# zilliztech/knowhere

Hardware: NVIDIA H100
Metric: queries/sec at recall@10>=0.95, 10Mx128 f32 IVF_PQ (higher is better)
Workload: dtype f32

## Files before the change

### knowhere_b200/csrc/kb2_ivfpq_tc.cuh

```cuda
#pragma once
#include <cuda_bf16.h>

#include <type_traits>
#include <utility>

#include "kb2_gemm_tc.cuh"
#include "kb2_ivf.cuh"
#include "kb2_listmajor.cuh"

namespace kb2 {
namespace pqtc {

using lm::TM;
constexpr int NQT = 256;
constexpr int THREADS = 512;
constexpr int GROUP_THREADS = 128;
constexpr int MAXW = 80;
constexpr int META_BYTES = 3 * NQT * 4;
template <int G, int DSUB>
struct TcCfg {
    static constexpr int M = 16 * G;
    static constexpr int KD = M * DSUB;
    static_assert(KD % 16 == 0 && (DSUB == 2 || DSUB == 4 || DSUB == 8), "unsupported PQ geometry");
    static constexpr int XCHUNK = KD / 8;
    static constexpr int KSTEPS = KD / 16 + 1;
    static constexpr int CHUNKS = 2 * KSTEPS;
    static constexpr int GRP_BYTES = CHUNKS * 128;
    static constexpr int TAB_BYTES = M * 256 * DSUB * 2;
    static constexpr int A_BYTES = (TM / 8) * GRP_BYTES, B_BYTES = (NQT / 8) * GRP_BYTES;
    static constexpr int OFF_TAB = 0;
    static constexpr int OFF_A = TAB_BYTES;
    static constexpr int OFF_B = OFF_A + 2 * A_BYTES;
    static constexpr int OFF_META = OFF_B + B_BYTES;
    static constexpr int OFF_BAR = OFF_META + 2 * META_BYTES;
    static constexpr size_t SMEM_BYTES = OFF_BAR + 256 + 128 ;
    static_assert(SMEM_BYTES <= 227 * 1024, "filter kernel shared memory");
};
constexpr int KD = 128;
constexpr float kErrCoef = 0.0085f;
constexpr float kAccCoef = 4e-5f;

struct Params {
    int metric;
    int nq, nprobe;
    const float* queries;
    const __nv_bfloat16* qb16;
    const float* qnorm;
    const int32_t* n_items;
    int32_t* ticket;
    const int32_t* item_list;
    const int32_t* item_q0;
    const int32_t* item_nq;
    const int32_t* pair_q;
    const float* pair_base;
    const float* bound;
    int k_need;
    float margin_coef;
    float rmax;
    const int64_t* list_off;
    const int32_t* list_len;
    const uint4* codes;
    const uint4* codes_plain;
    int64_t npad;
    const float* t1;
    const float* pqc;
    const uint4* pqc16;
    const uint8_t* bitset;
    const int32_t* rows;
    uint4* log;
    uint32_t* log_cnt;
    uint32_t log_cap;
    uint32_t* qflag;
    unsigned long long* counters;
};

template <typename F, int... I>
__device__ __forceinline__ void
static_for_impl(F&& f, std::integer_sequence<int, I...>) {
    (f(std::integral_constant<int, I>{}), ...);
}
template <int N, typename F>
__device__ __forceinline__ void
static_for(F&& f) {
    static_for_impl(f, std::make_integer_sequence<int, N>{});
}
template <int C0_, int W_>
struct BlockCols {
    static constexpr int C0 = C0_, W = W_;
};
template <int LO, int HI, typename F>
__device__ __forceinline__ void
dispatch_range(int n, F&& f) {
    if constexpr (LO == HI) {
        f(std::integral_constant<int, LO>{});
    } else {
        constexpr int MID = (LO + HI) / 2;
        if (n <= MID) dispatch_range<LO, MID>(n, f);
        else dispatch_range<MID + 1, HI>(n, f);
    }
}

__device__ __forceinline__ void
bar_sync_epi() {
    asm volatile("bar.sync 1, 256;" ::: "memory");
}
__device__ __forceinline__ uint64_t
make_desc_ns(uint32_t smem_addr, uint32_t grp_bytes) {
    uint64_t d = 0;
    d |= (uint64_t)((smem_addr & 0x3FFFFu) >> 4);
    d |= (uint64_t)(128 >> 4) << 16;
    d |= (uint64_t)(grp_bytes >> 4) << 32;
    return d;
}

#ifdef KB2_FILTER_STALLS
#define KB2_STALL_BEGIN(v) const long long v = clock64()
#define KB2_STALL_END(slot, v) stall[slot] += clock64() - (v)
constexpr int kStallMaxCtas = 1024, kStallSlots = 8;
__device__ unsigned long long g_filter_stalls[kStallMaxCtas][2][2][kStallSlots];
__global__ void
filter_stalls_print_kernel(int ctas) {
    for (int b = 0; b < min(ctas, kStallMaxCtas); b++) {
        printf("KB2STALL cta=%d", b);
        for (int r = 0; r < 2; r++) {
            printf(r == 0 ? " dec=" : " cons=");
            for (int i = 0; i < kStallSlots; i++)
                printf(i ? ",%llu" : "%llu", g_filter_stalls[b][r][0][i] + g_filter_stalls[b][r][1][i]);
        }
        printf("\n");
    }
}
#else
#define KB2_STALL_BEGIN(v)
#define KB2_STALL_END(slot, v)
#endif

__device__ __forceinline__ void
split3_bf16(float x, uint32_t& hi, uint32_t& mid, uint32_t& lo) {
    const __nv_bfloat16 h = __float2bfloat16_rn(x);
    hi = (uint32_t)__bfloat16_as_ushort(h);
    if (!(fabsf(x) < INFINITY)) { mid = 0u; lo = 0u; return; }
    const float r1 = x - __bfloat162float(h);
    const __nv_bfloat16 m = __float2bfloat16_rn(r1);
    const float r2 = r1 - __bfloat162float(m);
    mid = (uint32_t)__bfloat16_as_ushort(m);
    lo = (uint32_t)__bfloat16_as_ushort(__float2bfloat16_rn(r2));
}

template <int METRIC, int G, int DSUB>
__global__ void __launch_bounds__(THREADS, 1)
ivfpq_tc_filter_kernel(Params p) {
    using C = TcCfg<G, DSUB>;
    constexpr int KD = C::KD, XCHUNK = C::XCHUNK, KSTEPS = C::KSTEPS, GRP_BYTES = C::GRP_BYTES, TAB_BYTES = C::TAB_BYTES;
    constexpr int A_BYTES = C::A_BYTES, OFF_TAB = C::OFF_TAB, OFF_A = C::OFF_A, OFF_B = C::OFF_B, OFF_META = C::OFF_META,
                  OFF_BAR = C::OFF_BAR;
    extern __shared__ unsigned char smem_dyn[];
    const uint32_t raw = tc::smem_u32(smem_dyn);
    const uint32_t base = (raw + 127u) & ~127u;
    unsigned char* sm = smem_dyn + (base - raw);
    const uint32_t bars = base + OFF_BAR;
    auto bar_a_full = [&](int i) { return bars + 8u * i; };
    auto bar_a_empty = [&](int i) { return bars + 8u * (2 + i); };
    const uint32_t bar_b_full = bars + 8u * 8, bar_b_free = bars + 8u * 9;
    auto bar_meta_full = [&](int i) { return bars + 8u * (10 + i); };
    auto bar_meta_free = [&](int i) { return bars + 8u * (12 + i); };
    uint32_t* qcnt = (uint32_t*)(sm + OFF_BAR + 8 * 15);

    const int warp = __shfl_sync(0xffffffffu, (int)threadIdx.x >> 5, 0), lane = threadIdx.x & 31;
    const int n_items = *p.n_items;

    const lm::ItemRing<8> ring(sm + OFF_BAR + 144, p.ticket);
    ring.init();

    if (threadIdx.x == 0) {
        for (int i = 0; i < 2; i++) {
            tc::mbar_init(bar_a_full(i), GROUP_THREADS);
            tc::mbar_init(bar_a_empty(i), GROUP_THREADS);
            tc::mbar_init(bar_meta_full(i), 2 * GROUP_THREADS);
            tc::mbar_init(bar_meta_free(i), 2 * GROUP_THREADS);
        }
        tc::mbar_init(bar_b_full, 2 * GROUP_THREADS);
        tc::mbar_init(bar_b_free, 2 * GROUP_THREADS);
        qcnt[0] = qcnt[1] = qcnt[2] = qcnt[3] = 0;
        asm volatile("fence.mbarrier_init.release.cluster;" ::: "memory");
    }
#ifdef KB2_FILTER_STALLS
    long long stall[kStallSlots] = {0, 0, 0, 0, 0, 0, 0, 0};
    KB2_STALL_BEGIN(t_role);
#endif
    {
        uint4* tab = (uint4*)(sm + OFF_TAB);
        for (int i = threadIdx.x; i < TAB_BYTES / 16; i += THREADS) tab[i] = __ldg(p.pqc16 + i);
    }
    __syncthreads();
    const float inv_alpha = (METRIC == KB2_METRIC_L2) ? 0.5f : 1.f;

    if (warp < 8) {
        const int dt = threadIdx.x;
        const int dg = dt >> 7;
        const int tid = dt & 127;
        const uint4* tab = (const uint4*)(sm + OFF_TAB);
        auto write_meta = [&](int item, int it) {
            KB2_STALL_BEGIN(t_meta);
            const int par = it & 1;
            tc::mbar_wait(bar_meta_free(par), (((uint32_t)it >> 1) & 1u) ^ 1u);
            const int q0 = p.item_q0[item];
            const int nqi = p.item_nq[item];
            float* m_h = (float*)(sm + OFF_META + par * META_BYTES);
            float* m_base = m_h + NQT;
            int* m_q = (int*)(m_base + NQT);
            const int j = dt;
            float h = -INFINITY, bs = 0.f;
            int q = -1;
            if (j < nqi) {
                q = p.pair_q[q0 + j];
                bs = p.pair_base[q0 + j];
                const float bnd = p.bound[q];
                if (!(bnd < INFINITY)) {
                    p.qflag[q] = 1u;
                    if (p.counters) atomicAdd(p.counters + 6, 1ull << 32);
                } else {
                    const float margin = p.margin_coef * p.qnorm[q] * 1.01f + 1e-30f;
                    const float h0 = (bnd + margin - bs) * inv_alpha;
                    h = h0 + kAccCoef * (fabsf(h0) + p.rmax) + 1e-30f;
                }
            }
            m_h[j] = h;
            m_base[j] = bs;
            m_q[j] = q;
            tc::mbar_arrive(bar_meta_full(par));
            KB2_STALL_END(5, t_meta);
        };
        uint32_t g0 = 0;
        int it = 0;
        int item = ring.at_warp(0);
        if (item < n_items) write_meta(item, 0);
        for (; item < n_items; it++) {
            const int item_next = ring.at_warp(it + 1);
            const int l = p.item_list[item];
            const int nqi = p.item_nq[item];
            const int nmma = (nqi + 15) & ~15;
            const int len = p.list_len[l];
            const int64_t off = p.list_off[l];
            const int ntiles = (len + TM - 1) / TM;
            const int par = it & 1;
            const int t_first = (int)((dg - (int)(g0 & 1u)) & 1);
            uint4 w_next[G];
#pragma unroll
            for (int g = 0; g < G; g++) w_next[g] = make_uint4(0, 0, 0, 0);
            float t_next = 0.f;
            const uint4* code_src = (DSUB == 8) ? p.codes : p.codes_plain;
            if (t_first < ntiles && off + (int64_t)t_first * TM + tid < p.npad) {
#pragma unroll
                for (int g = 0; g < G; g++) w_next[g] = ldg_stream_u4(code_src + (int64_t)g * p.npad + off + (int64_t)t_first * TM + tid);
                if (METRIC == KB2_METRIC_L2) t_next = __ldg(p.t1 + off + (int64_t)t_first * TM + tid);
            }
            auto decode_tile = [&](int t) {
                KB2_STALL_BEGIN(t_dec);
                const uint32_t g = g0 + (uint32_t)t;
                uint4 w[G];
#pragma unroll
                for (int gg = 0; gg < G; gg++) w[gg] = w_next[gg];
                const float tv = t_next;
                {
                    const int64_t pn = off + (int64_t)(t + 2) * TM + tid;
                    if (t + 2 < ntiles && pn < p.npad) {
#pragma unroll
                        for (int gg = 0; gg < G; gg++) w_next[gg] = ldg_stream_u4(code_src + (int64_t)gg * p.npad + pn);
                        if (METRIC == KB2_METRIC_L2) t_next = __ldg(p.t1 + pn);
                    }
                }
                float r = INFINITY;
                if (t * TM + tid < len) r = (METRIC == KB2_METRIC_L2) ? 0.5f * tv : 0.f;
                uint32_t rh, rm, rl;
                split3_bf16(-r, rh, rm, rl);
                uint4 v[XCHUNK];
                if constexpr (DSUB == 8) {
#pragma unroll
                    for (int gg = 0; gg < G; gg++) {
                        const uint32_t ww[4] = {w[gg].x, w[gg].y, w[gg].z, w[gg].w};
#pragma unroll
                        for (int s = 0; s < 16; s++) {
                            const uint32_t byte = (ww[s >> 2] >> (8 * (s & 3))) & 255u;
                            v[gg * 16 + s] = tab[byte * (16 * G) + gg * 16 + ((s + tid) & 15)];
                        }
                    }
                } else {
                    constexpr int SPC = 8 / DSUB;
                    constexpr int WPS = DSUB / 2;
                    const uint32_t* tab32 = reinterpret_cast<const uint32_t*>(tab);
#pragma unroll
                    for (int c = 0; c < XCHUNK; c++) {
                        uint32_t u[4];
#pragma unroll
                        for (int j = 0; j < SPC; j++) {
                            const int m = c * SPC + j;
                            const uint4 wg = w[m >> 4];
                            const int b = m & 15;
                            const uint32_t word = (b < 4) ? wg.x : (b < 8) ? wg.y : (b < 12) ? wg.z : wg.w;
                            const uint32_t byte = (word >> (8 * (b & 3))) & 255u;
#pragma unroll
                            for (int x = 0; x < WPS; x++) u[j * WPS + x] = tab32[(m * 256 + byte) * WPS + x];
                        }
                        v[c] = make_uint4(u[0], u[1], u[2], u[3]);
                    }
                }
                KB2_STALL_BEGIN(t_ae);
                tc::mbar_wait(bar_a_empty(dg), ((g >> 1) & 1u) ^ 1u);
                KB2_STALL_END(1, t_ae);
                unsigned char* A = sm + OFF_A + dg * A_BYTES + (tid >> 3) * GRP_BYTES + (tid & 7) * 16;
#pragma unroll
                for (int c = 0; c < XCHUNK; c++) {
                    const int chunk = (DSUB == 8) ? (c & ~15) + ((c + tid) & 15) : c;
                    *reinterpret_cast<uint4*>(A + chunk * 128) = v[c];
                }
                *reinterpret_cast<uint4*>(A + XCHUNK * 128) = make_uint4(rh | (rm << 16), rl | (0x3F80u << 16), 0x3F803F80u, 0u);
                *reinterpret_cast<uint4*>(A + (XCHUNK + 1) * 128) = make_uint4(0u, 0u, 0u, 0u);
                tc::fence_proxy_async();
                tc::mbar_arrive(bar_a_full(dg));
                KB2_STALL_END(3, t_dec);
            };
            if (t_first < ntiles) decode_tile(t_first);
            KB2_STALL_BEGIN(t_b);
            asm volatile("bar.sync 2, 256;" ::: "memory");
            KB2_STALL_BEGIN(t_bf);
            tc::mbar_wait(bar_b_free, ((uint32_t)it & 1u) ^ 1u);
            KB2_STALL_END(2, t_bf);
            {
                const float* m_h = (const float*)(sm + OFF_META + par * META_BYTES);
                const int* m_q = (const int*)(m_h + 2 * NQT);
                const uint32_t Bs = base + OFF_B;
                unsigned char* B = sm + OFF_B;
                const int kc = tid >> 3;
                const int rsub = tid & 7;
                for (int blk = dg; blk < nmma / 8 && kc < XCHUNK; blk += 2) {
                    const int row = blk * 8 + rsub;
                    const int q = m_q[row];
                    const uint32_t dst = (uint32_t)(blk * GRP_BYTES + kc * 128 + rsub * 16);
                    if (q >= 0) {
                        const void* src = reinterpret_cast<const uint4*>(p.qb16 + (int64_t)q * KD) + kc;
                        asm volatile("cp.async.cg.shared.global [%0], [%1], 16;" ::"r"(Bs + dst), "l"(src) : "memory");
                    } else {
                        *reinterpret_cast<uint4*>(B + dst) = make_uint4(0, 0, 0, 0);
                    }
                }
                if (dt < nmma) {
                    uint32_t hh, hm, hl;
                    split3_bf16(m_h[dt], hh, hm, hl);
                    unsigned char* Bc = B + (dt >> 3) * GRP_BYTES + (dt & 7) * 16;
                    *reinterpret_cast<uint4*>(Bc + XCHUNK * 128) = make_uint4(0x3F803F80u, 0x3F80u | (hh << 16), hm | (hl << 16), 0u);
                    *reinterpret_cast<uint4*>(Bc + (XCHUNK + 1) * 128) = make_uint4(0u, 0u, 0u, 0u);
                }
                asm volatile("cp.async.wait_all;" ::: "memory");
            }
            tc::fence_proxy_async();
            tc::mbar_arrive(bar_b_full);
            KB2_STALL_END(4, t_b);
            if (item_next < n_items) write_meta(item_next, it + 1);
            for (int t = t_first + 2; t < ntiles; t += 2) decode_tile(t);
            g0 += (uint32_t)ntiles;
            item = item_next;
        }
    } else {
        const int et = threadIdx.x - 256;
        const int eg = et >> 7;
        const int e = et & 127;
        const int we = warp & 3;
        const uint32_t n_logs = 2u * gridDim.x;
        uint4* my_log = p.log + (size_t)(2 * blockIdx.x + eg) * p.log_cap;
        uint32_t* my_cursor = qcnt + eg;
        bool log_over = false;
        unsigned long long n_codes = 0;
        uint32_t g0 = 0;
        int it = 0;
        for (int item = ring.at_warp(0); item < n_items; item = ring.at_warp(++it)) {
            const int l = p.item_list[item];
            const int nqi = p.item_nq[item];
            const int ncls = __shfl_sync(0xffffffffu, (nqi + 15) >> 4, 0);
            const int len = p.list_len[l];
            const int64_t off = p.list_off[l];
            const int ntiles = (len + TM - 1) / TM;
            const int par = it & 1;
            KB2_STALL_BEGIN(t_mf);
            tc::mbar_wait(bar_meta_full(par), ((uint32_t)it >> 1) & 1u);
            KB2_STALL_END(1, t_mf);
            const float* m_base = (const float*)(sm + OFF_META + par * META_BYTES) + NQT;
            const int* m_q = (const int*)(m_base + NQT);
            if (et == 0) n_codes += (unsigned long long)len * (unsigned long long)nqi;
            const int t_first = (int)((eg - (int)(g0 & 1u)) & 1);
            KB2_STALL_BEGIN(t_bfull);
            tc::mbar_wait(bar_b_full, (uint32_t)it & 1u);
            KB2_STALL_END(2, t_bfull);
            const uint32_t a0 = base + OFF_A + eg * A_BYTES;
            const uint32_t b0 = base + OFF_B;
            const uint32_t la0 = (uint32_t)make_desc_ns(a0, GRP_BYTES), lb0 = (uint32_t)make_desc_ns(b0, GRP_BYTES);
            constexpr uint64_t desc_hi = (uint64_t)(GRP_BYTES >> 4) << 32;
            for (int t = t_first; t < ntiles; t += 2) {
                const uint32_t g = g0 + (uint32_t)t;
                KB2_STALL_BEGIN(t_af);
                tc::mbar_wait(bar_a_full(eg), (g >> 1) & 1u);
                KB2_STALL_END(3, t_af);
                auto issue = [&](auto& acc, int h, auto blk) {
                    using B = decltype(blk);
                    KB2_STALL_BEGIN(t_is);
                    uint32_t la = la0 + (uint32_t)(h * 8 * GRP_BYTES / 16), lb = lb0 + (uint32_t)(B::C0 / 8 * GRP_BYTES / 16);
                    if constexpr (G == 1) asm volatile("" : "+r"(la), "+r"(lb));
                    tc::fence_operand(acc);
                    tc::wgmma_fence();
#pragma unroll
                    for (int ks = 0; ks < KSTEPS; ks++)
                        tc::wgmma_bf16<B::W>(acc, desc_hi | (la + ks * 16u), desc_hi | (lb + ks * 16u), ks > 0 ? 1u : 0u);
                    tc::wgmma_commit();
                    tc::fence_operand(acc);
                    KB2_STALL_END(6, t_is);
                };
                uint64_t mh[2][2] = {{0ull, 0ull}, {0ull, 0ull}};
                auto test = [&](const auto& v, int h, auto blk) {
                    using B = decltype(blk);
                    constexpr int NBIT = B::W / 4, HALF = NBIT / 2;
                    KB2_STALL_BEGIN(t_te);
                    uint32_t n0l = 0u, n0h = 0u, n1l = 0u, n1h = 0u;
#pragma unroll
                    for (int i = HALF - 1; i >= 0; i--) {
                        const int x = 4 * (i >> 1) + (i & 1);
                        const int xh = 4 * ((i + HALF) >> 1) + ((i + HALF) & 1);
                        n0l = __funnelshift_l(__float_as_uint(v[x]), n0l, 1);
                        n0h = __funnelshift_l(__float_as_uint(v[xh]), n0h, 1);
                        n1l = __funnelshift_l(__float_as_uint(v[x + 2]), n1l, 1);
                        n1h = __funnelshift_l(__float_as_uint(v[xh + 2]), n1h, 1);
                    }
                    constexpr uint32_t mask = (1u << NBIT) - 1u;
                    const uint32_t m0 = ~((n0h << HALF) | n0l) & mask, m1 = ~((n1h << HALF) | n1l) & mask;
                    mh[h][0] |= (uint64_t)m0 << (B::C0 / 4);
                    mh[h][1] |= (uint64_t)m1 << (B::C0 / 4);
                    KB2_STALL_END(7, t_te);
                };
                auto flush = [&]() {
                    const uint32_t total =
                        (uint32_t)(__popcll(mh[0][0]) + __popcll(mh[0][1]) + __popcll(mh[1][0]) + __popcll(mh[1][1]));
                    if (total != 0u) {
                        uint32_t slot = atomicAdd(my_cursor, total);
#pragma unroll
                        for (int h = 0; h < 2; h++) {
#pragma unroll
                            for (int i = 0; i < 2; i++) {
                                const int rel = t * TM + h * 64 + we * 16 + (lane >> 2) + 8 * i;
                                uint64_t m = mh[h][i];
                                while (m) {
                                    const int bit = __ffsll((long long)m) - 1;
                                    m &= m - 1;
                                    const int col = 8 * (bit >> 1) + 2 * (lane & 3) + (bit & 1);
                                    if (slot < p.log_cap) {
                                        uint4 o;
                                        o.x = (uint32_t)m_q[col];
                                        o.y = (uint32_t)(off + rel);
                                        o.z = __float_as_uint(m_base[col]);
                                        o.w = 0u;
                                        my_log[slot] = o;
                                    } else {
                                        log_over = true;
                                    }
                                    slot++;
                                }
                            }
                        }
                    }
                };
                dispatch_range<1, NQT / 16>(ncls, [&](auto nc) {
                    constexpr int NC = decltype(nc)::value, NB = (16 * NC + MAXW - 1) / MAXW, NBT = 2 * NB;
                    constexpr int U = NC / NB, X = NC % NB;
                    auto blk = [](auto cc) {
                        constexpr int c = decltype(cc)::value;
                        return BlockCols<16 * (c * U + (c < X ? c : X)), 16 * (U + (c < X ? 1 : 0))>{};
                    };
                    float va[8 * (U + (X > 0 ? 1 : 0))], vb[8 * (U + (X > 0 ? 1 : 0))];
                    issue(va, 0, blk(std::integral_constant<int, 0>{}));
                    static_for<NBT>([&](auto bc) {
                        constexpr int b = decltype(bc)::value;
                        if constexpr (b + 1 < NBT) {
                            constexpr auto bn = blk(std::integral_constant<int, (b + 1) % NB>{});
                            if constexpr ((b + 1) & 1) issue(vb, (b + 1) / NB, bn);
                            else issue(va, (b + 1) / NB, bn);
                            KB2_STALL_BEGIN(t_w);
                            tc::wgmma_wait<1>();
                            KB2_STALL_END(4, t_w);
                        } else {
                            KB2_STALL_BEGIN(t_w);
                            tc::wgmma_wait<0>();
                            KB2_STALL_END(4, t_w);
                        }
                        constexpr auto bb = blk(std::integral_constant<int, b % NB>{});
                        if constexpr (b & 1) {
                            tc::fence_operand(vb);
                            test(vb, b / NB, bb);
                        } else {
                            tc::fence_operand(va);
                            test(va, b / NB, bb);
                        }
                    });
                });
                tc::mbar_arrive(bar_a_empty(eg));
                KB2_STALL_BEGIN(t_fl);
                flush();
                KB2_STALL_END(5, t_fl);
            }
            tc::mbar_arrive(bar_b_free);
            tc::mbar_arrive(bar_meta_free(par));
            g0 += (uint32_t)ntiles;
        }
        if (log_over) p.log_cnt[n_logs] = 1u;
        if (eg == 0) asm volatile("bar.sync 3, 128;" ::: "memory"); else asm volatile("bar.sync 4, 128;" ::: "memory");
        if (e == 0) {
            const uint32_t n = min(*my_cursor, p.log_cap);
            p.log_cnt[2 * blockIdx.x + eg] = n;
            if (p.counters) atomicAdd(p.counters + 2, (unsigned long long)n);
        }
        if (et == 0 && p.counters) atomicAdd(p.counters, n_codes);
    }
#ifdef KB2_FILTER_STALLS
    KB2_STALL_END(0, t_role);
    if ((threadIdx.x & 127) == 0 && blockIdx.x < kStallMaxCtas) {
        for (int i = 0; i < kStallSlots; i++)
            g_filter_stalls[blockIdx.x][warp >= 8][(threadIdx.x >> 7) & 1][i] = (unsigned long long)stall[i];
    }
#endif
}

__global__ void
prepare_queries_kernel(const float* __restrict__ q, int64_t nq, int d, __nv_bfloat16* __restrict__ qb16, float* __restrict__ qnorm) {
    const int64_t w = ((int64_t)blockIdx.x * blockDim.x + threadIdx.x) >> 5;
    const int lane = threadIdx.x & 31;
    if (w >= nq) return;
    float s = 0.f;
    for (int j = lane * 4; j < d; j += 128) {
        const float4 v = __ldg(reinterpret_cast<const float4*>(q + w * d + j));
        __nv_bfloat162 lo = __floats2bfloat162_rn(v.x, v.y), hi = __floats2bfloat162_rn(v.z, v.w);
        uint2 o;
        o.x = *reinterpret_cast<uint32_t*>(&lo);
        o.y = *reinterpret_cast<uint32_t*>(&hi);
        *reinterpret_cast<uint2*>(qb16 + w * d + j) = o;
        s += v.x * v.x + v.y * v.y + v.z * v.z + v.w * v.w;
    }
    s = warp_sum(s);
    if (lane == 0) qnorm[w] = sqrtf(s) * 1.0001f;
}

__global__ void __launch_bounds__(256)
prepare_tables_kernel(const float* __restrict__ pqc, int dsub, __nv_bfloat16* __restrict__ pqc16, float* __restrict__ maxn2) {
    const int m = blockIdx.x, j = threadIdx.x;
    const int M = gridDim.x;
    const float* c = pqc + ((size_t)m * 256 + j) * dsub;
    float n2 = 0.f;
    __nv_bfloat16* o = pqc16 + (dsub == 8 ? ((size_t)j * M + m) : ((size_t)m * 256 + j)) * dsub;
    for (int t = 0; t < dsub; t++) {
        n2 = fmaf(c[t], c[t], n2);
        o[t] = __float2bfloat16_rn(c[t]);
    }
    __shared__ float red[256];
    red[j] = n2;
    __syncthreads();
    for (int s = 128; s > 0; s >>= 1) {
        if (j < s) red[j] = fmaxf(red[j], red[j + s]);
        __syncthreads();
    }
    if (j == 0) maxn2[m] = red[0];
}
__global__ void
unrotate_codes_kernel(const uint8_t* __restrict__ rot, int64_t total_words , int64_t npad, uint8_t* __restrict__ plain) {
    const int64_t t = (int64_t)blockIdx.x * blockDim.x + threadIdx.x;
    if (t >= total_words * 16) return;
    const int s = (int)(t & 15);
    const int64_t word = t >> 4;
    const int64_t pos = word % npad;
    plain[word * 16 + ((s + (int)(pos & 15)) & 15)] = rot[t];
}

template <int METRIC>
__global__ void __launch_bounds__(256, 1)
lut_build_kernel(const float* __restrict__ queries, int64_t nq, const int32_t* __restrict__ qlist, const uint32_t* __restrict__ qcount,
                 const float* __restrict__ pqc, float* __restrict__ lut) {
    __shared__ __align__(16) float s_q[2][KD];
    const int j = threadIdx.x;
    const float scale = (METRIC == KB2_METRIC_L2) ? -2.f : -1.f;
    if (qlist) nq = (int64_t)*qcount;
    float4 c[32];
#pragma unroll
    for (int m = 0; m < 16; m++) {
        const float* cp = pqc + ((size_t)m * 256 + j) * 8;
        c[2 * m] = __ldg(reinterpret_cast<const float4*>(cp));
        c[2 * m + 1] = __ldg(reinterpret_cast<const float4*>(cp + 4));
    }
    const int64_t per = (nq + gridDim.x - 1) / gridDim.x;
    const int64_t q_beg = (int64_t)blockIdx.x * per, q_end = min(nq, q_beg + per);
    auto qrow = [&](int64_t i) { return queries + (qlist ? (int64_t)qlist[i] : i) * KD; };
    if (q_beg < q_end && threadIdx.x < KD) s_q[0][threadIdx.x] = qrow(q_beg)[threadIdx.x];
    __syncthreads();
    for (int64_t q = q_beg; q < q_end; q++) {
        const int cur = (int)((q - q_beg) & 1);
        if (q + 1 < q_end && threadIdx.x < KD) s_q[cur ^ 1][threadIdx.x] = qrow(q + 1)[threadIdx.x];
        float* dst = lut + q * 4096 + j * 16;
#pragma unroll
        for (int m4 = 0; m4 < 16; m4 += 4) {
            float o[4];
#pragma unroll
            for (int u = 0; u < 4; u++) {
                const int m = m4 + u;
                const float4 qa = *reinterpret_cast<const float4*>(&s_q[cur][m * 8]);
                const float4 qb = *reinterpret_cast<const float4*>(&s_q[cur][m * 8 + 4]);
                float a = 0.f;
                a = fmaf(qa.x, c[2 * m].x, a); a = fmaf(qa.y, c[2 * m].y, a); a = fmaf(qa.z, c[2 * m].z, a); a = fmaf(qa.w, c[2 * m].w, a);
                a = fmaf(qb.x, c[2 * m + 1].x, a); a = fmaf(qb.y, c[2 * m + 1].y, a); a = fmaf(qb.z, c[2 * m + 1].z, a); a = fmaf(qb.w, c[2 * m + 1].w, a);
                o[u] = a * scale;
            }
            *reinterpret_cast<float4*>(dst + m4) = make_float4(o[0], o[1], o[2], o[3]);
        }
        __syncthreads();
    }
}

template <int METRIC, int G, int DSUB>
__global__ void __launch_bounds__(128)
exact_eval_kernel(const float* __restrict__ queries, const float* __restrict__ pqc, const float* __restrict__ lut,
                  const float* __restrict__ bound_of,
                  const uint4* __restrict__ codes, int64_t npad, const float* __restrict__ t1, const uint8_t* __restrict__ bitset,
                  const int32_t* __restrict__ rows, uint64_t* __restrict__ cand, uint32_t* __restrict__ cand_cnt, int cap,
                  uint32_t* __restrict__ qflag, const uint32_t* __restrict__ log_over, int k_trim = 0) {
    constexpr int KDIM = 16 * G * DSUB;
    __shared__ __align__(16) float s_q[KDIM];
    __shared__ uint32_t s_h[256];
    __shared__ float s_red[8];
    __shared__ uint32_t s_ctl[2];
    const int64_t q = blockIdx.x;
    if (*log_over) {
        if (threadIdx.x == 0) qflag[q] = 1u;
        return;
    }
    if (qflag[q]) return;
    const uint32_t n = min(cand_cnt[q], (uint32_t)cap);
    if (n == 0) return;
    const bool use_lut = (G == 1 && DSUB == 8) && lut != nullptr;
    if (!use_lut) {
        for (int j = threadIdx.x; j < KDIM; j += 128) s_q[j] = queries[q * KDIM + j];
        __syncthreads();
    }
    const float* lq = lut + q * 4096;
    const float bound = bound_of[q];
    const float scale = (METRIC == KB2_METRIC_L2) ? -2.f : -1.f;
    uint64_t* row = cand + q * cap;
    auto eval = [&](uint64_t ent, float& key_out) -> uint64_t {
        const uint32_t pos = (uint32_t)ent;
        const float base = __uint_as_float((uint32_t)(ent >> 32));
        float acc0 = (METRIC == KB2_METRIC_L2) ? __ldg(t1 + pos) : 0.f, acc1 = 0.f;
#pragma unroll
        for (int g = 0; g < G; g++) {
            const uint4 w = __ldg(codes + (int64_t)g * npad + pos);
            const uint32_t ww[4] = {w.x, w.y, w.z, w.w};
#pragma unroll
            for (int s = 0; s < 16; s++) {
                const uint32_t byte = (ww[s >> 2] >> (8 * (s & 3))) & 255u;
                const uint32_t m = g * 16 + ((pos + s) & 15u);
                float v;
                if (use_lut) {
                    v = __ldg(lq + byte * 16 + m);
                } else {
                    const float* c = pqc + ((size_t)m * 256 + byte) * DSUB;
                    const float* qs = &s_q[m * DSUB];
                    float a = 0.f;
#pragma unroll
                    for (int t = 0; t < DSUB; t++) a = fmaf(qs[t], __ldg(c + t), a);
                    v = __fmul_rn(a, scale);
                }
                if (s & 1) acc1 = __fadd_rn(acc1, v); else acc0 = __fadd_rn(acc0, v);
            }
        }
        const float key = __fadd_rn(base, __fadd_rn(acc0, acc1));
        bool keep = key <= bound;
        if (keep && bitset) keep = !bit_is_set(bitset, rows[pos]);
        key_out = keep ? key : INFINITY;
        return keep ? pack_kp(key, pos) : kEmpty;
    };
    if (k_trim > 0 && n <= 512u && n > (uint32_t)k_trim) {
        uint64_t pk[4];
        float kf[4];
        float lo = INFINITY, hi = -INFINITY;
        s_h[threadIdx.x] = 0;
        s_h[threadIdx.x + 128] = 0;
        if (threadIdx.x == 0) s_ctl[1] = 0;
#pragma unroll
        for (int it = 0; it < 4; it++) {
            const uint32_t i = threadIdx.x + it * 128;
            pk[it] = kEmpty;
            kf[it] = INFINITY;
            if (i < n) pk[it] = eval(row[i], kf[it]);
            if (kf[it] < INFINITY) { lo = fminf(lo, kf[it]); hi = fmaxf(hi, kf[it]); }
        }
#pragma unroll
        for (int o = 16; o > 0; o >>= 1) {
            lo = fminf(lo, __shfl_xor_sync(0xffffffffu, lo, o));
            hi = fmaxf(hi, __shfl_xor_sync(0xffffffffu, hi, o));
        }
        if ((threadIdx.x & 31) == 0) { s_red[threadIdx.x >> 5] = lo; s_red[4 + (threadIdx.x >> 5)] = hi; }
        __syncthreads();
        lo = fminf(fminf(s_red[0], s_red[1]), fminf(s_red[2], s_red[3]));
        hi = fmaxf(fmaxf(s_red[4], s_red[5]), fmaxf(s_red[6], s_red[7]));
        const float sc = (hi > lo) ? 256.f / (hi - lo) : 0.f;
        int bin[4];
#pragma unroll
        for (int it = 0; it < 4; it++) {
            bin[it] = 256;
            if (kf[it] < INFINITY) {
                bin[it] = min(255, (int)((kf[it] - lo) * sc));
                atomicAdd(&s_h[bin[it]], 1u);
            }
        }
        __syncthreads();
        if (threadIdx.x < 32) {
            const int lane = threadIdx.x;
            uint32_t h[8], sum = 0;
#pragma unroll
            for (int t = 0; t < 8; t++) { h[t] = s_h[lane * 8 + t]; sum += h[t]; }
            uint32_t incl = sum;
#pragma unroll
            for (int o = 1; o < 32; o <<= 1) {
                const uint32_t v = __shfl_up_sync(0xffffffffu, incl, o);
                if (lane >= o) incl += v;
            }
            const uint32_t excl = incl - sum;
            const uint32_t total = __shfl_sync(0xffffffffu, incl, 31);
            if (lane == 0 && total < (uint32_t)k_trim) s_ctl[0] = 255u;
            if (excl < (uint32_t)k_trim && incl >= (uint32_t)k_trim) {
                uint32_t run = excl;
                int b = lane * 8 + 7;
#pragma unroll
                for (int t = 0; t < 8; t++) {
                    run += h[t];
                    if (run >= (uint32_t)k_trim) { b = lane * 8 + t; break; }
                }
                s_ctl[0] = (uint32_t)b;
            }
        }
        __syncthreads();
        const int bstar = (int)s_ctl[0];
#pragma unroll
        for (int it = 0; it < 4; it++)
            if (bin[it] <= bstar) row[atomicAdd(&s_ctl[1], 1u)] = pk[it];
        __syncthreads();
        if (threadIdx.x == 0) cand_cnt[q] = s_ctl[1];
        return;
    }
    float lo = INFINITY, hi = -INFINITY;
    for (uint32_t i = threadIdx.x; i < n; i += 128) {
        float kf;
        row[i] = eval(row[i], kf);
        if (kf < INFINITY) { lo = fminf(lo, kf); hi = fmaxf(hi, kf); }
    }
    if (k_trim > 0 && k_trim <= 96 && n > 512u) {
        __shared__ uint64_t s_stage[128];
        s_h[threadIdx.x] = 0;
        s_h[threadIdx.x + 128] = 0;
        if (threadIdx.x == 0) { s_ctl[0] = 0xffffffffu; s_ctl[1] = 0; }
#pragma unroll
        for (int o = 16; o > 0; o >>= 1) {
            lo = fminf(lo, __shfl_xor_sync(0xffffffffu, lo, o));
            hi = fmaxf(hi, __shfl_xor_sync(0xffffffffu, hi, o));
        }
        if ((threadIdx.x & 31) == 0) { s_red[threadIdx.x >> 5] = lo; s_red[4 + (threadIdx.x >> 5)] = hi; }
        __syncthreads();
        lo = fminf(fminf(s_red[0], s_red[1]), fminf(s_red[2], s_red[3]));
        hi = fmaxf(fmaxf(s_red[4], s_red[5]), fmaxf(s_red[6], s_red[7]));
        const float sc = (hi > lo) ? 256.f / (hi - lo) : 0.f;
        for (uint32_t i = threadIdx.x; i < n; i += 128) {
            const uint64_t e = row[i];
            if (e != kEmpty) atomicAdd(&s_h[min(255, (int)((unpack_key(e) - lo) * sc))], 1u);
        }
        __syncthreads();
        if (threadIdx.x < 32) {
            const int lane = threadIdx.x;
            uint32_t h[8], sum = 0;
#pragma unroll
            for (int t = 0; t < 8; t++) { h[t] = s_h[lane * 8 + t]; sum += h[t]; }
            uint32_t incl = sum;
#pragma unroll
            for (int o = 1; o < 32; o <<= 1) {
                const uint32_t v = __shfl_up_sync(0xffffffffu, incl, o);
                if (lane >= o) incl += v;
            }
            const uint32_t excl = incl - sum;
            if (excl < (uint32_t)k_trim && incl >= (uint32_t)k_trim) {
                uint32_t run = excl;
                int b = lane * 8 + 7;
#pragma unroll
                for (int t = 0; t < 8; t++) {
                    run += h[t];
                    if (run >= (uint32_t)k_trim) { b = lane * 8 + t; break; }
                }
                if (run <= 128u) s_ctl[0] = (uint32_t)b;
            }
        }
        __syncthreads();
        const uint32_t bstar = s_ctl[0];
        if (bstar == 0xffffffffu) return;
        for (uint32_t i = threadIdx.x; i < n; i += 128) {
            const uint64_t e = row[i];
            if (e != kEmpty && (uint32_t)min(255, (int)((unpack_key(e) - lo) * sc)) <= bstar) s_stage[atomicAdd(&s_ctl[1], 1u)] = e;
        }
        __syncthreads();
        const uint32_t nk = s_ctl[1];
        for (uint32_t i = threadIdx.x; i < nk; i += 128) row[i] = s_stage[i];
        if (threadIdx.x == 0) cand_cnt[q] = nk;
    }
}

__global__ void __launch_bounds__(1024)
compact_resp_kernel(const int64_t* __restrict__ probe_ids, int nprobe, int64_t nq, const int32_t* __restrict__ list_owner, int rank,
                    int32_t* __restrict__ list, uint32_t* __restrict__ count) {
    __shared__ uint32_t s_n;
    if (threadIdx.x == 0) s_n = 0;
    __syncthreads();
    for (int64_t q = threadIdx.x; q < nq; q += 1024) {
        const int64_t l = probe_ids[q * nprobe];
        if (l >= 0 && list_owner[l] == rank) list[atomicAdd(&s_n, 1u)] = (int32_t)q;
    }
    __syncthreads();
    if (threadIdx.x == 0) *count = s_n;
}
__global__ void
fill_f32_kernel(float* __restrict__ out, int64_t n, float v) {
    const int64_t i = (int64_t)blockIdx.x * blockDim.x + threadIdx.x;
    if (i < n) out[i] = v;
}
__global__ void __launch_bounds__(256)
max_abs_kernel(const float* __restrict__ x, int64_t n, uint32_t* __restrict__ out) {
    float m = 0.f;
    for (int64_t i = (int64_t)blockIdx.x * blockDim.x + threadIdx.x; i < n; i += (int64_t)gridDim.x * blockDim.x) m = fmaxf(m, fabsf(x[i]));
#pragma unroll
    for (int o = 16; o > 0; o >>= 1) m = fmaxf(m, __shfl_xor_sync(0xffffffffu, m, o));
    if ((threadIdx.x & 31) == 0 && m > 0.f) atomicMax(out, __float_as_uint(m));
}

__global__ void __launch_bounds__(1024)
compact_flags_kernel(const uint32_t* __restrict__ qflag, int64_t nq, int32_t* __restrict__ list, uint32_t* __restrict__ count) {
    __shared__ uint32_t s_n;
    if (threadIdx.x == 0) s_n = 0;
    __syncthreads();
    for (int64_t q = threadIdx.x; q < nq; q += 1024)
        if (qflag[q]) list[atomicAdd(&s_n, 1u)] = (int32_t)q;
    __syncthreads();
    if (threadIdx.x == 0) *count = s_n;
}

#define KB2_BOUND_STEP(WORD, KB, S, ACC)                                                      \
    {                                                                                         \
        const uint32_t _x = __byte_perm((WORD), lane4, 0x6504u | ((KB) << 4));                \
        float _v;                                                                             \
        asm("ld.shared.f32 %0, [%1+%2];" : "=f"(_v) : "r"(_x >> 1), "n"(KB2_SMEM_BASE + 4 * (S))); \
        ACC += _v;                                                                            \
    }
__global__ void
transpose_codebook_kernel(const float* __restrict__ pqc, int M, int dsub, float* __restrict__ pqc_t) {
    const int64_t i = (int64_t)blockIdx.x * blockDim.x + threadIdx.x;
    const int64_t n = (int64_t)M * 256 * dsub;
    if (i >= n) return;
    const int x = (int)(i % dsub);
    const int j = (int)((i / dsub) % 256);
    const int m = (int)(i / ((int64_t)dsub * 256));
    pqc_t[((((int64_t)(m >> 4) * 256 + j) * 16) + (m & 15)) * dsub + x] = pqc[i];
}
constexpr int BOUND_KMAX = 6144;
constexpr int BOUND_BINS = 1024;
__host__ __device__ constexpr int bound_kmax(int min_codes, int k_need) {
    const int want = ((min_codes > k_need ? min_codes : k_need) + 63) & ~63;
    return want < BOUND_KMAX ? want : BOUND_KMAX;
}
constexpr size_t bound_smem(int kmax) { return (size_t)32 * 1024 + (size_t)kmax * 4 + BOUND_BINS * 4 + 128; }

template <int METRIC, int G, int DSUB, int NT>
__global__ void __launch_bounds__(NT)
bound_kernel(const float* __restrict__ lut, const int32_t* __restrict__ qlist, const uint32_t* __restrict__ qcount, int64_t nq,
             const int64_t* __restrict__ probe_ids, const float* __restrict__ probe_dis,
             int probe_stride, int p0_max, int min_codes, int k_need, const int64_t* __restrict__ list_off,
             const int32_t* __restrict__ list_len, const uint4* __restrict__ codes, const float* __restrict__ t1,
             const uint8_t* __restrict__ bitset, const int32_t* __restrict__ rows, float* __restrict__ out,
             unsigned long long* __restrict__ counters, int64_t npad = 0, const float* __restrict__ queries = nullptr,
             const float* __restrict__ pqc_t = nullptr) {
    static_assert(NT == 128 || NT == 256, "bound_kernel block size");
    constexpr int NW = NT / 32;
    constexpr int BPT = BOUND_BINS / NT;
    extern __shared__ __align__(16) unsigned char smem_raw[];
    float* s_lut = (float*)smem_raw;
    const int key_cap = bound_kmax(min_codes, k_need);
    float* s_keys = (float*)(smem_raw + 32 * 1024);
    uint32_t* s_hist = (uint32_t*)(s_keys + key_cap);
    float* s_red = (float*)(s_hist + BOUND_BINS);
    const int warp = threadIdx.x >> 5, lane = threadIdx.x & 31;
    if ((uint32_t)__cvta_generic_to_shared(smem_raw) != (uint32_t)KB2_SMEM_BASE) {
        if (threadIdx.x == 0 && counters) atomicExch(counters + 1, 0xBAD5ull);
        return;
    }
    const int64_t n_work = qlist ? (int64_t)*qcount : nq;
    for (int64_t wi = blockIdx.x; wi < n_work; wi += gridDim.x) {
    const int64_t q = qlist ? (int64_t)qlist[wi] : wi;
    int seen = 0, n_tot = 0;
    float kmin = INFINITY, kmax = -INFINITY;
#pragma unroll 1
    for (int g = 0; g < G; g++) {
    __syncthreads();
    if constexpr (G > 1 || DSUB != 8) {
        const float scale = (METRIC == KB2_METRIC_L2) ? -2.f : -1.f;
        const int mm = threadIdx.x & 15, jsub = threadIdx.x >> 4;
        float qv[DSUB];
#pragma unroll
        for (int x = 0; x < DSUB; x++) qv[x] = queries[q * (int64_t)(16 * G * DSUB) + (g * 16 + mm) * DSUB + x];
        for (int j = jsub; j < 256; j += NT / 16) {
            const float* cp = pqc_t + (((size_t)g * 256 + j) * 16 + mm) * DSUB;
            float a = 0.f;
#pragma unroll
            for (int x = 0; x < DSUB; x++) a = fmaf(qv[x], __ldg(cp + x), a);
            a *= scale;
            s_lut[j * 32 + mm] = a;
            s_lut[j * 32 + 16 + mm] = a;
        }
    } else {
        const float4* src = reinterpret_cast<const float4*>(lut + wi * 4096);
#pragma unroll
        for (int i = 0; i < 1024 / NT; i++) {
            const int idx = threadIdx.x + i * NT;
            const float4 v = __ldg(src + idx);
            float4* dst = reinterpret_cast<float4*>(s_lut + (idx >> 2) * 32 + (idx & 3) * 4);
            dst[0] = v;
            dst[4] = v;
        }
    }
    if (g == 0)
        for (int i = threadIdx.x; i < BOUND_BINS; i += NT) s_hist[i] = 0;
    __syncthreads();
    const uint32_t lane4 = (uint32_t)(lane & 15) << 3;
    const uint4* gcodes = codes + (int64_t)g * npad;
    const bool first_g = (g == 0), last_g = (g == G - 1);
    seen = 0;
    n_tot = 0;
    const int code_cap = min(key_cap, max(min_codes, k_need));
    for (int j = 0; j < p0_max && seen < min_codes && n_tot < code_cap; j++) {
        const int64_t l = probe_ids[q * probe_stride + j];
        if (l < 0) continue;
        const int len_all = list_len[l];
        if (len_all == 0) continue;
        seen += len_all;
        const int len = min(len_all, code_cap - n_tot);
        const int64_t off = list_off[l];
        const float dv = probe_dis[q * probe_stride + j];
        const float base = (METRIC == KB2_METRIC_L2) ? dv : -dv;
        uint4 nA = make_uint4(0, 0, 0, 0), nB = nA;
        float ntA = 0.f, ntB = 0.f;
        auto load_iter = [&](int c0) {
            if (c0 < len) {
                nA = ldg_stream_u4(gcodes + off + c0 + lane);
                if (METRIC == KB2_METRIC_L2 && first_g) ntA = __ldg(t1 + off + c0 + lane);
                if (c0 + 32 < len) {
                    nB = ldg_stream_u4(gcodes + off + c0 + 32 + lane);
                    if (METRIC == KB2_METRIC_L2 && first_g) ntB = __ldg(t1 + off + c0 + 32 + lane);
                }
            }
        };
        load_iter(warp * 64);
        for (int c0 = warp * 64; c0 < len; c0 += NW * 64) {
            const int relA = c0 + lane, relB = c0 + 32 + lane;
            const bool okA = relA < len, okB = relB < len;
            const uint32_t posA = (uint32_t)(off + relA), posB = (uint32_t)(off + relB);
            const bool hasB = c0 + 32 < len;
            const uint4 wA = nA;
            const uint4 wB = hasB ? nB : nA;
            float a0 = ntA, a1 = 0.f, b0 = hasB ? ntB : 0.f, b1 = 0.f;
            load_iter(c0 + NW * 64);
            KB2_BOUND_STEP(wA.x, 0, 0, a0)  KB2_BOUND_STEP(wB.x, 0, 0, b0)  KB2_BOUND_STEP(wA.x, 1, 1, a1)  KB2_BOUND_STEP(wB.x, 1, 1, b1)
            KB2_BOUND_STEP(wA.x, 2, 2, a0)  KB2_BOUND_STEP(wB.x, 2, 2, b0)  KB2_BOUND_STEP(wA.x, 3, 3, a1)  KB2_BOUND_STEP(wB.x, 3, 3, b1)
            KB2_BOUND_STEP(wA.y, 0, 4, a0)  KB2_BOUND_STEP(wB.y, 0, 4, b0)  KB2_BOUND_STEP(wA.y, 1, 5, a1)  KB2_BOUND_STEP(wB.y, 1, 5, b1)
            KB2_BOUND_STEP(wA.y, 2, 6, a0)  KB2_BOUND_STEP(wB.y, 2, 6, b0)  KB2_BOUND_STEP(wA.y, 3, 7, a1)  KB2_BOUND_STEP(wB.y, 3, 7, b1)
            KB2_BOUND_STEP(wA.z, 0, 8, a0)  KB2_BOUND_STEP(wB.z, 0, 8, b0)  KB2_BOUND_STEP(wA.z, 1, 9, a1)  KB2_BOUND_STEP(wB.z, 1, 9, b1)
            KB2_BOUND_STEP(wA.z, 2, 10, a0) KB2_BOUND_STEP(wB.z, 2, 10, b0) KB2_BOUND_STEP(wA.z, 3, 11, a1) KB2_BOUND_STEP(wB.z, 3, 11, b1)
            KB2_BOUND_STEP(wA.w, 0, 12, a0) KB2_BOUND_STEP(wB.w, 0, 12, b0) KB2_BOUND_STEP(wA.w, 1, 13, a1) KB2_BOUND_STEP(wB.w, 1, 13, b1)
            KB2_BOUND_STEP(wA.w, 2, 14, a0) KB2_BOUND_STEP(wB.w, 2, 14, b0) KB2_BOUND_STEP(wA.w, 3, 15, a1) KB2_BOUND_STEP(wB.w, 3, 15, b1)
            float keyA = (first_g ? base : s_keys[n_tot + (okA ? relA : 0)]) + (a0 + a1);
            float keyB = (first_g ? base : s_keys[n_tot + ((hasB && okB) ? relB : 0)]) + (b0 + b1);
            if (okA) {
                if (last_g && bitset && bit_is_set(bitset, rows[posA])) keyA = INFINITY;
                s_keys[n_tot + relA] = keyA;
                if (last_g && keyA < INFINITY) { kmin = fminf(kmin, keyA); kmax = fmaxf(kmax, keyA); }
            }
            if (hasB && okB) {
                if (last_g && bitset && bit_is_set(bitset, rows[posB])) keyB = INFINITY;
                s_keys[n_tot + relB] = keyB;
                if (last_g && keyB < INFINITY) { kmin = fminf(kmin, keyB); kmax = fmaxf(kmax, keyB); }
            }
        }
        n_tot += len;
    }
    }
#pragma unroll
    for (int o = 16; o > 0; o >>= 1) {
        kmin = fminf(kmin, __shfl_xor_sync(0xffffffffu, kmin, o));
        kmax = fmaxf(kmax, __shfl_xor_sync(0xffffffffu, kmax, o));
    }
    if (lane == 0) { s_red[warp] = kmin; s_red[8 + warp] = kmax; }
    __syncthreads();
    float lo = s_red[0], hi = s_red[8];
#pragma unroll
    for (int w = 1; w < NW; w++) { lo = fminf(lo, s_red[w]); hi = fmaxf(hi, s_red[8 + w]); }
    const float scale = (hi > lo) ? (float)BOUND_BINS / (hi - lo) : 0.f;
    for (int i = threadIdx.x; i < n_tot; i += NT) {
        const float kv = s_keys[i];
        if (kv < INFINITY) atomicAdd(&s_hist[min(BOUND_BINS - 1, (int)((kv - lo) * scale))], 1u);
    }
    __syncthreads();
    uint32_t mine[BPT], tsum = 0;
#pragma unroll
    for (int b = 0; b < BPT; b++) { mine[b] = s_hist[threadIdx.x * BPT + b]; tsum += mine[b]; }
    uint32_t incl = tsum;
#pragma unroll
    for (int o = 1; o < 32; o <<= 1) {
        const uint32_t v = __shfl_up_sync(0xffffffffu, incl, o);
        if (lane >= o) incl += v;
    }
    uint32_t* s_wsum = (uint32_t*)(s_red + 16);
    if (lane == 31) s_wsum[warp] = incl;
    __syncthreads();
    uint32_t before = incl - tsum;
    for (int w = 0; w < warp; w++) before += s_wsum[w];
    uint32_t total = 0;
#pragma unroll
    for (int w = 0; w < NW; w++) total += s_wsum[w];
    const uint32_t need = (uint32_t)k_need;
    if (total < need || seen < 4 * k_need) {
        if (threadIdx.x == 0) out[q] = INFINITY;
    } else if (before < need && before + tsum >= need) {
        uint32_t cum = before;
        int b = 0;
#pragma unroll
        for (int bb = 0; bb < BPT; bb++) {
            if (cum < need) { cum += mine[bb]; b = bb; }
        }
        const float bound = (scale > 0.f) ? lo + ((float)(threadIdx.x * BPT + b) + 1.01f) / scale : hi;
        out[q] = fmaxf(bound, lo) + (G == 1 ? 4e-7f : 2e-6f) * fmaxf(fabsf(lo), fabsf(hi));
    }
    }
}
#undef KB2_BOUND_STEP

}
}
```

Before: 4.224 million.

## Use a single decoder warpgroup with double-buffered loads, cutting block to 384 threads

The kernel drops from two decoder warpgroups to one, so blocks have 384 threads instead of 512. The remaining decoder group handles every tile in sequence, using a two-deep register prefetch of code rows, and loops over the meta and B-tile rows the second group used to cover. MAXW is raised from 80 to 128, which widens the consumer's column blocks. The code-count atomic moves to the decoder side, the log-overflow flag is written directly, and the list offset becomes 32-bit. The aim is to free registers and threads for more resident blocks or larger tiles, at the cost of halving decode parallelism, which may starve the wgmma consumers.

Result: no change. 4.282 million (median of 6 runs) (+1.4%).

```diff
diff --git a/knowhere_b200/csrc/kb2_ivfpq_tc.cuh b/knowhere_b200/csrc/kb2_ivfpq_tc.cuh
--- a/knowhere_b200/csrc/kb2_ivfpq_tc.cuh
+++ b/knowhere_b200/csrc/kb2_ivfpq_tc.cuh
@@ -13,9 +13,9 @@
 
 using lm::TM;
 constexpr int NQT = 256;
-constexpr int THREADS = 512;
+constexpr int THREADS = 384;
 constexpr int GROUP_THREADS = 128;
-constexpr int MAXW = 80;
+constexpr int MAXW = 128;
 constexpr int META_BYTES = 3 * NQT * 4;
 template <int G, int DSUB>
 struct TcCfg {
@@ -117,16 +117,14 @@
 #define KB2_STALL_BEGIN(v) const long long v = clock64()
 #define KB2_STALL_END(slot, v) stall[slot] += clock64() - (v)
 constexpr int kStallMaxCtas = 1024, kStallSlots = 8;
-__device__ unsigned long long g_filter_stalls[kStallMaxCtas][2][2][kStallSlots];
+__device__ unsigned long long g_filter_stalls[kStallMaxCtas][THREADS / 128][kStallSlots];
 __global__ void
 filter_stalls_print_kernel(int ctas) {
     for (int b = 0; b < min(ctas, kStallMaxCtas); b++) {
-        printf("KB2STALL cta=%d", b);
-        for (int r = 0; r < 2; r++) {
-            printf(r == 0 ? " dec=" : " cons=");
-            for (int i = 0; i < kStallSlots; i++)
-                printf(i ? ",%llu" : "%llu", g_filter_stalls[b][r][0][i] + g_filter_stalls[b][r][1][i]);
-        }
+        printf("KB2STALL cta=%d dec=", b);
+        for (int i = 0; i < kStallSlots; i++) printf(i ? ",%llu" : "%llu", g_filter_stalls[b][0][i]);
+        printf(" cons=");
+        for (int i = 0; i < kStallSlots; i++) printf(i ? ",%llu" : "%llu", g_filter_stalls[b][1][i] + g_filter_stalls[b][2][i]);
         printf("\n");
     }
 }
@@ -176,10 +174,10 @@
         for (int i = 0; i < 2; i++) {
             tc::mbar_init(bar_a_full(i), GROUP_THREADS);
             tc::mbar_init(bar_a_empty(i), GROUP_THREADS);
-            tc::mbar_init(bar_meta_full(i), 2 * GROUP_THREADS);
+            tc::mbar_init(bar_meta_full(i), GROUP_THREADS);
             tc::mbar_init(bar_meta_free(i), 2 * GROUP_THREADS);
         }
-        tc::mbar_init(bar_b_full, 2 * GROUP_THREADS);
+        tc::mbar_init(bar_b_full, GROUP_THREADS);
         tc::mbar_init(bar_b_free, 2 * GROUP_THREADS);
         qcnt[0] = qcnt[1] = qcnt[2] = qcnt[3] = 0;
         asm volatile("fence.mbarrier_init.release.cluster;" ::: "memory");
@@ -195,10 +193,8 @@
     __syncthreads();
     const float inv_alpha = (METRIC == KB2_METRIC_L2) ? 0.5f : 1.f;
 
-    if (warp < 8) {
-        const int dt = threadIdx.x;
-        const int dg = dt >> 7;
-        const int tid = dt & 127;
+    if (warp < 4) {
+        const int tid = threadIdx.x;
         const uint4* tab = (const uint4*)(sm + OFF_TAB);
         auto write_meta = [&](int item, int it) {
             KB2_STALL_BEGIN(t_meta);
@@ -209,29 +205,32 @@
             float* m_h = (float*)(sm + OFF_META + par * META_BYTES);
             float* m_base = m_h + NQT;
             int* m_q = (int*)(m_base + NQT);
-            const int j = dt;
-            float h = -INFINITY, bs = 0.f;
-            int q = -1;
-            if (j < nqi) {
-                q = p.pair_q[q0 + j];
-                bs = p.pair_base[q0 + j];
-                const float bnd = p.bound[q];
-                if (!(bnd < INFINITY)) {
-                    p.qflag[q] = 1u;
-                    if (p.counters) atomicAdd(p.counters + 6, 1ull << 32);
-                } else {
-                    const float margin = p.margin_coef * p.qnorm[q] * 1.01f + 1e-30f;
-                    const float h0 = (bnd + margin - bs) * inv_alpha;
-                    h = h0 + kAccCoef * (fabsf(h0) + p.rmax) + 1e-30f;
+#pragma unroll
+            for (int j = tid; j < NQT; j += GROUP_THREADS) {
+                float h = -INFINITY, bs = 0.f;
+                int q = -1;
+                if (j < nqi) {
+                    q = p.pair_q[q0 + j];
+                    bs = p.pair_base[q0 + j];
+                    const float bnd = p.bound[q];
+                    if (!(bnd < INFINITY)) {
+                        p.qflag[q] = 1u;
+                        if (p.counters) atomicAdd(p.counters + 6, 1ull << 32);
+                    } else {
+                        const float margin = p.margin_coef * p.qnorm[q] * 1.01f + 1e-30f;
+                        const float h0 = (bnd + margin - bs) * inv_alpha;
+                        h = h0 + kAccCoef * (fabsf(h0) + p.rmax) + 1e-30f;
+                    }
                 }
-            }
-            m_h[j] = h;
-            m_base[j] = bs;
-            m_q[j] = q;
+                m_h[j] = h;
+                m_base[j] = bs;
+                m_q[j] = q;
+            }
             tc::mbar_arrive(bar_meta_full(par));
             KB2_STALL_END(5, t_meta);
         };
         uint32_t g0 = 0;
+        unsigned long long n_codes = 0;
         int it = 0;
         int item = ring.at_warp(0);
         if (item < n_items) write_meta(item, 0);
@@ -244,32 +243,35 @@
             const int64_t off = p.list_off[l];
             const int ntiles = (len + TM - 1) / TM;
             const int par = it & 1;
-            const int t_first = (int)((dg - (int)(g0 & 1u)) & 1);
-            uint4 w_next[G];
-#pragma unroll
-            for (int g = 0; g < G; g++) w_next[g] = make_uint4(0, 0, 0, 0);
-            float t_next = 0.f;
+            if (tid == 0) n_codes += (unsigned long long)len * (unsigned long long)nqi;
             const uint4* code_src = (DSUB == 8) ? p.codes : p.codes_plain;
-            if (t_first < ntiles && off + (int64_t)t_first * TM + tid < p.npad) {
-#pragma unroll
-                for (int g = 0; g < G; g++) w_next[g] = ldg_stream_u4(code_src + (int64_t)g * p.npad + off + (int64_t)t_first * TM + tid);
-                if (METRIC == KB2_METRIC_L2) t_next = __ldg(p.t1 + off + (int64_t)t_first * TM + tid);
-            }
+            uint4 w0[G], w1[G];
+            float t0 = 0.f, t1v = 0.f;
+            auto load_row = [&](int t, uint4 (&w)[G], float& tv) {
+                const int64_t pn = off + (int64_t)t * TM + tid;
+                if (t < ntiles && pn < p.npad) {
+#pragma unroll
+                    for (int gg = 0; gg < G; gg++) w[gg] = ldg_stream_u4(code_src + (int64_t)gg * p.npad + pn);
+                    if (METRIC == KB2_METRIC_L2) tv = __ldg(p.t1 + pn);
+                }
+            };
+#pragma unroll
+            for (int g = 0; g < G; g++) w0[g] = w1[g] = make_uint4(0, 0, 0, 0);
+            load_row(0, w0, t0);
+            load_row(1, w1, t1v);
             auto decode_tile = [&](int t) {
                 KB2_STALL_BEGIN(t_dec);
                 const uint32_t g = g0 + (uint32_t)t;
+                const int ab = (int)(g & 1u);
                 uint4 w[G];
 #pragma unroll
-                for (int gg = 0; gg < G; gg++) w[gg] = w_next[gg];
-                const float tv = t_next;
-                {
-                    const int64_t pn = off + (int64_t)(t + 2) * TM + tid;
-                    if (t + 2 < ntiles && pn < p.npad) {
-#pragma unroll
-                        for (int gg = 0; gg < G; gg++) w_next[gg] = ldg_stream_u4(code_src + (int64_t)gg * p.npad + pn);
-                        if (METRIC == KB2_METRIC_L2) t_next = __ldg(p.t1 + pn);
-                    }
+                for (int gg = 0; gg < G; gg++) {
+                    w[gg] = w0[gg];
+                    w0[gg] = w1[gg];
                 }
+                const float tv = t0;
+                t0 = t1v;
+                load_row(t + 2, w1, t1v);
                 float r = INFINITY;
                 if (t * TM + tid < len) r = (METRIC == KB2_METRIC_L2) ? 0.5f * tv : 0.f;
                 uint32_t rh, rm, rl;
@@ -306,9 +308,9 @@
                     }
                 }
                 KB2_STALL_BEGIN(t_ae);
-                tc::mbar_wait(bar_a_empty(dg), ((g >> 1) & 1u) ^ 1u);
+                tc::mbar_wait(bar_a_empty(ab), ((g >> 1) & 1u) ^ 1u);
                 KB2_STALL_END(1, t_ae);
-                unsigned char* A = sm + OFF_A + dg * A_BYTES + (tid >> 3) * GRP_BYTES + (tid & 7) * 16;
+                unsigned char* A = sm + OFF_A + ab * A_BYTES + (tid >> 3) * GRP_BYTES + (tid & 7) * 16;
 #pragma unroll
                 for (int c = 0; c < XCHUNK; c++) {
                     const int chunk = (DSUB == 8) ? (c & ~15) + ((c + tid) & 15) : c;
@@ -317,12 +319,13 @@
                 *reinterpret_cast<uint4*>(A + XCHUNK * 128) = make_uint4(rh | (rm << 16), rl | (0x3F80u << 16), 0x3F803F80u, 0u);
                 *reinterpret_cast<uint4*>(A + (XCHUNK + 1) * 128) = make_uint4(0u, 0u, 0u, 0u);
                 tc::fence_proxy_async();
-                tc::mbar_arrive(bar_a_full(dg));
+                tc::mbar_arrive(bar_a_full(ab));
                 KB2_STALL_END(3, t_dec);
             };
-            if (t_first < ntiles) decode_tile(t_first);
+            int t = 0;
+            for (; t < 2 && t < ntiles; t++) decode_tile(t);
             KB2_STALL_BEGIN(t_b);
-            asm volatile("bar.sync 2, 256;" ::: "memory");
+            asm volatile("bar.sync 2, 128;" ::: "memory");
             KB2_STALL_BEGIN(t_bf);
             tc::mbar_wait(bar_b_free, ((uint32_t)it & 1u) ^ 1u);
             KB2_STALL_END(2, t_bf);
@@ -333,7 +336,7 @@
                 unsigned char* B = sm + OFF_B;
                 const int kc = tid >> 3;
                 const int rsub = tid & 7;
-                for (int blk = dg; blk < nmma / 8 && kc < XCHUNK; blk += 2) {
+                for (int blk = 0; blk < nmma / 8 && kc < XCHUNK; blk++) {
                     const int row = blk * 8 + rsub;
                     const int q = m_q[row];
                     const uint32_t dst = (uint32_t)(blk * GRP_BYTES + kc * 128 + rsub * 16);
@@ -344,10 +347,10 @@
                         *reinterpret_cast<uint4*>(B + dst) = make_uint4(0, 0, 0, 0);
                     }
                 }
-                if (dt < nmma) {
+                for (int j = tid; j < nmma; j += GROUP_THREADS) {
                     uint32_t hh, hm, hl;
-                    split3_bf16(m_h[dt], hh, hm, hl);
-                    unsigned char* Bc = B + (dt >> 3) * GRP_BYTES + (dt & 7) * 16;
+                    split3_bf16(m_h[j], hh, hm, hl);
+                    unsigned char* Bc = B + (j >> 3) * GRP_BYTES + (j & 7) * 16;
                     *reinterpret_cast<uint4*>(Bc + XCHUNK * 128) = make_uint4(0x3F803F80u, 0x3F80u | (hh << 16), hm | (hl << 16), 0u);
                     *reinterpret_cast<uint4*>(Bc + (XCHUNK + 1) * 128) = make_uint4(0u, 0u, 0u, 0u);
                 }
@@ -357,20 +360,19 @@
             tc::mbar_arrive(bar_b_full);
             KB2_STALL_END(4, t_b);
             if (item_next < n_items) write_meta(item_next, it + 1);
-            for (int t = t_first + 2; t < ntiles; t += 2) decode_tile(t);
+            for (; t < ntiles; t++) decode_tile(t);
             g0 += (uint32_t)ntiles;
             item = item_next;
         }
+        if (tid == 0 && p.counters) atomicAdd(p.counters, n_codes);
     } else {
-        const int et = threadIdx.x - 256;
+        const int et = threadIdx.x - GROUP_THREADS;
         const int eg = et >> 7;
         const int e = et & 127;
         const int we = warp & 3;
         const uint32_t n_logs = 2u * gridDim.x;
         uint4* my_log = p.log + (size_t)(2 * blockIdx.x + eg) * p.log_cap;
         uint32_t* my_cursor = qcnt + eg;
-        bool log_over = false;
-        unsigned long long n_codes = 0;
         uint32_t g0 = 0;
         int it = 0;
         for (int item = ring.at_warp(0); item < n_items; item = ring.at_warp(++it)) {
@@ -378,7 +380,7 @@
             const int nqi = p.item_nq[item];
             const int ncls = __shfl_sync(0xffffffffu, (nqi + 15) >> 4, 0);
             const int len = p.list_len[l];
-            const int64_t off = p.list_off[l];
+            const uint32_t off = (uint32_t)p.list_off[l];
             const int ntiles = (len + TM - 1) / TM;
             const int par = it & 1;
             KB2_STALL_BEGIN(t_mf);
@@ -386,7 +388,6 @@
             KB2_STALL_END(1, t_mf);
             const float* m_base = (const float*)(sm + OFF_META + par * META_BYTES) + NQT;
             const int* m_q = (const int*)(m_base + NQT);
-            if (et == 0) n_codes += (unsigned long long)len * (unsigned long long)nqi;
             const int t_first = (int)((eg - (int)(g0 & 1u)) & 1);
             KB2_STALL_BEGIN(t_bfull);
             tc::mbar_wait(bar_b_full, (uint32_t)it & 1u);
@@ -404,7 +405,7 @@
                     using B = decltype(blk);
                     KB2_STALL_BEGIN(t_is);
                     uint32_t la = la0 + (uint32_t)(h * 8 * GRP_BYTES / 16), lb = lb0 + (uint32_t)(B::C0 / 8 * GRP_BYTES / 16);
-                    if constexpr (G == 1) asm volatile("" : "+r"(la), "+r"(lb));
+                    asm volatile("" : "+r"(la), "+r"(lb));
                     tc::fence_operand(acc);
                     tc::wgmma_fence();
 #pragma unroll
@@ -429,7 +430,7 @@
                         n1l = __funnelshift_l(__float_as_uint(v[x + 2]), n1l, 1);
                         n1h = __funnelshift_l(__float_as_uint(v[xh + 2]), n1h, 1);
                     }
-                    constexpr uint32_t mask = (1u << NBIT) - 1u;
+                    constexpr uint32_t mask = NBIT < 32 ? (1u << (NBIT & 31)) - 1u : ~0u;
                     const uint32_t m0 = ~((n0h << HALF) | n0l) & mask, m1 = ~((n1h << HALF) | n1l) & mask;
                     mh[h][0] |= (uint64_t)m0 << (B::C0 / 4);
                     mh[h][1] |= (uint64_t)m1 << (B::C0 / 4);
@@ -453,12 +454,12 @@
                                     if (slot < p.log_cap) {
                                         uint4 o;
                                         o.x = (uint32_t)m_q[col];
-                                        o.y = (uint32_t)(off + rel);
+                                        o.y = off + (uint32_t)rel;
                                         o.z = __float_as_uint(m_base[col]);
                                         o.w = 0u;
                                         my_log[slot] = o;
                                     } else {
-                                        log_over = true;
+                                        p.log_cnt[n_logs] = 1u;
                                     }
                                     slot++;
                                 }
@@ -508,20 +509,17 @@
             tc::mbar_arrive(bar_meta_free(par));
             g0 += (uint32_t)ntiles;
         }
-        if (log_over) p.log_cnt[n_logs] = 1u;
         if (eg == 0) asm volatile("bar.sync 3, 128;" ::: "memory"); else asm volatile("bar.sync 4, 128;" ::: "memory");
         if (e == 0) {
             const uint32_t n = min(*my_cursor, p.log_cap);
             p.log_cnt[2 * blockIdx.x + eg] = n;
             if (p.counters) atomicAdd(p.counters + 2, (unsigned long long)n);
         }
-        if (et == 0 && p.counters) atomicAdd(p.counters, n_codes);
     }
 #ifdef KB2_FILTER_STALLS
     KB2_STALL_END(0, t_role);
     if ((threadIdx.x & 127) == 0 && blockIdx.x < kStallMaxCtas) {
-        for (int i = 0; i < kStallSlots; i++)
-            g_filter_stalls[blockIdx.x][warp >= 8][(threadIdx.x >> 7) & 1][i] = (unsigned long long)stall[i];
+        for (int i = 0; i < kStallSlots; i++) g_filter_stalls[blockIdx.x][threadIdx.x >> 7][i] = (unsigned long long)stall[i];
     }
 #endif
 }
```
